# leejaehot/GaussianGrasper

Measured on AMD Instinct MI355X. Metric: rendered views/sec (fwd+bwd) at 1M Gaussians, 1600x1200, 32-ch feature, higher is better.
Workload: dtype f32; 1 GPU; BASELINE config 4 per-GPU share: 1000000 Gaussians, 1600x1200, SH deg 4 rgb + 32-ch feature + depth + normal images per view (nerfstudio plugin route: the timed callable is FusedGaussianSplattingModel.get_outputs(camera) of gaussiangrasper_amd.plugin (the class train.sh loads, on stub.py's stand-ins for nerfstudio's base model and Cameras) — one fused rasterize operator per view), fwd+bwd, 8 views; route=plugin, deterministic_backward=False, python_gc=gc.freeze() after the warm-up (bench.freeze_gc), view_pipeline=backward of view k beside forward of view k + 1 on two streams, num_gaussians=1000000, feature_dim=32, n_visible=992125, parallelism=view-parallel x1, replicated Gaussians, grad_allreduce_bytes=472000000, grad_allreduce=per parameter, overlapped with the last view's backward

## Files before the change

### gaussiangrasper_amd/_lib.py

```python
from __future__ import annotations

import ctypes as C
import os

_HERE = os.path.dirname(os.path.abspath(__file__))
LIB_PATH = os.path.join(_HERE, "libgg_raster.so")
ABI_VERSION = 6

_P, _I, _F, _I64, _SZ = C.c_void_p, C.c_int, C.c_float, C.c_int64, C.c_size_t


class RowArray(C.Structure):
    _fields_ = [("src", C.c_void_p), ("dst", C.c_void_p), ("row_floats", C.c_int), ("kind", C.c_int)]


class AdamGroup(C.Structure):
    _fields_ = [("param", C.c_void_p), ("grad", C.c_void_p), ("exp_avg", C.c_void_p),
                ("exp_avg_sq", C.c_void_p), ("numel", C.c_int64), ("lr", C.c_double),
                ("beta1", C.c_double), ("beta2", C.c_double), ("eps", C.c_double),
                ("weight_decay", C.c_double), ("step", C.c_int64)]


ROWS_COPY, ROWS_MEANS, ROWS_SCALES, ROWS_ZERO_NEW = 0, 1, 2, 3
MAX_ROW_ARRAYS, ADAM_MAX_GROUPS = 24, 8
# ... 12 lines not shown
                               _P, _I, _P, _P, _P]),
    "gg_sh_fwd": (_I, [_I, _I, _I, _P, _P, _P, _P]),
    "gg_sh_bwd": (_I, [_I, _I, _I, _P, _P, _P, _P]),
    "gg_sh_bwd_accumulate": (_I, [_I, _I, _I, _P, _P, _P, _P]),
    "gg_quat_to_rotmat_fwd": (_I, [_I, _P, _P, _P]),
    "gg_quat_to_rotmat_bwd": (_I, [_I, _P, _P, _P, _P]),
    "gg_activate_fwd": (_I, [_I] + [_P] * 12),
    "gg_activate_bwd": (_I, [_I] + [_P] * 12),
    "gg_activate_bwd_ex": (_I, [_I] + [_P] * 7 + [_I] + [_P] * 4 + [_I, _P]),
    "gg_mlp_fwd": (_I, [_I64, _I, _I, _I, _P, _P, _P, _P, _P, _P, _P]),
    "gg_debug_set_fwd_blocks": (_I, [_I, _I]),
    "gg_mlp_fwd_fast_workspace": (_SZ, [_I, _I, _I]),
    "gg_mlp_fwd_fast": (_I, [_I64, _I, _I, _I, _P, _P, _P, _P, _P, _P, _P, _SZ, _P]),
    "gg_mlp_bwd": (_I, [_I64, _I, _I, _I] + [_P] * 11),
    "gg_cosine_loss_fwd": (_I, [_I64, _I, _P, _P, _P, _P, _P, _P, _P]),
    "gg_cosine_loss_bwd": (_I, [_I64, _I, _P, _P, _P, _P, _P, _P, _P, _P, _P]),
    "gg_count_workspace": (_SZ, [_I]),
    "gg_count_intersects": (_I, [_I, _P, _P, _P, _SZ, _P]),
    "gg_bin_sort_workspace": (_SZ, [_I, _I64]),
    "gg_bin_sort": (_I, [_I, _I64, _P, _P, _P, _P, _I, _I, _P, _P, _P, _P, _SZ, _P]),
    "gg_bin_sort_status": (_I, [_I, _I64, _P, _SZ, _P]),
    "gg_bin_sort_dev": (_I, [_I, _I64, _P, _P, _P, _P, _P, _I, _I, _P, _P, _P, _P, _SZ, _P]),
    "gg_bin_sort_dev_ex": (_I, [_I, _I64, _P, _P, _P, _P, _P, _I, _I, _P, _P, _P, _P, _SZ, _P, _P, _I, _P]),
    "gg_view_fwd_workspace": (_SZ, [_I]),
    "gg_view_fwd": (_I, [_I, _P, _P, _P, _P, _P, _P, _P, _F, _F, _F, _F, _I, _I, _I, _I, _F] + [_P] * 11 +
                    [_P, _P, _SZ, _P, _SZ, _P]),
    "gg_blend_fwd_pair_packed": (_I, [_I, _I, _I, _I, _I] + [_P] * 11 + [_SZ, _I, _P]),
    "gg_blend_workspace": (_SZ, [_I]),
    "gg_blend_fwd": (_I, [_I, _I, _I, _I, _P, _P, _P, _P, _P, _P, _P, _P, _P, _P, _P, _SZ, _P]),
    "gg_blend_fwd_pair": (_I, [_I, _I, _I, _I, _I] + [_P] * 14 + [_SZ, _P]),
    "gg_blend_fwd_pair_fast": (_I, [_I, _I, _I, _I, _I] + [_P] * 14 + [_SZ, _P]),
    "gg_blend_bwd": (_I, [_I, _I, _I, _I] + [_P] * 14 + [_I, _I, _P, _SZ, _I, _P]),
    "gg_shade_tail_bwd_split": (_I, [_I, _P, _I, _P, _P, _P, _P, _P]),
    "gg_view_bwd": (_I, [_I, _P, _I, _P, _P, _P, _F, _P, _P, _P, _P, _P, _P, _F, _F, _I, _I, _P, _P, _P, _P, _P, _P, _P, _P]),
    "gg_pose_grad_workspace": (_SZ, [_I]),
    "gg_view_bwd_pose": (_I, [_I, _P, _I, _P, _P, _P, _F, _P, _P, _P, _P, _P, _P, _F, _F, _I, _I] + [_P] * 9
                         + [_P, _SZ, _P]),
    "gg_project_pose_bwd": (_I, [_I, _P, _P, _F, _P, _P, _P, _F, _F, _I, _I, _P, _P, _P, _I, _P, _P, _I, _P, _P, _P,
                                 _SZ, _P]),
    "gg_sh_bwd_multi": (_I, [_I, _I, _I, _I, C.POINTER(_P), C.POINTER(_P), _P, _I, _P]),
    "gg_image_loss_workspace": (_SZ, [_I, _I]),
    "gg_image_loss_fwd": (_I, [_I, _I, _P, _I, _P, _P, _F, _P, _P, _SZ, _P]),
    "gg_image_loss_bwd": (_I, [_I, _I, _P, _I, _P, _P, _F, _P, _P, _SZ, _P, _P]),
    "gg_geom_loss_workspace": (_SZ, []),
    "gg_geom_loss_fwd": (_I, [_I64, _P, _I, _P, _I, _P, _I, _I, _P, _I, _I, _P, _P, _P, _SZ, _P]),
    "gg_geom_loss_bwd": (_I, [_I64, _P, _I, _P, _I, _P, _I, _I, _P, _I, _I, _P, _P, _P, _P, _SZ, _P, _P, _P]),
# ... 101 lines not shown
```

### gaussiangrasper_amd/csrc/binning.hip

```cpp
#include "scan.h"

__device__ __forceinline__ int64_t dev_count(int64_t n, const int64_t *__restrict__ n_dev) {
    if (n_dev) {
        const int64_t d = *n_dev;
        if (d < n) n = d;
    }
    return n;
}

#define RS_THREADS 256
#define RS_WAVES (RS_THREADS / GG_WAVE)
#ifndef GG_RS_BIG
#define GG_RS_BIG 16
#endif
static inline int rs_items(int64_t n) { return n >= (int64_t)4096 * 1024 ? GG_RS_BIG : 4; }

__global__ __launch_bounds__(256) void count_kernel(int N, const int32_t *__restrict__ nth,
                                                    unsigned long long *__restrict__ out) {
    __shared__ unsigned long long part[4];
    unsigned long long acc = 0;
    for (int i = blockIdx.x * blockDim.x + threadIdx.x; i < N; i += gridDim.x * blockDim.x)
        acc += (unsigned long long)(uint32_t)nth[i];
    for (int off = 32; off > 0; off >>= 1) acc += __shfl_down(acc, off, 64);
    if ((threadIdx.x & 63) == 0) part[threadIdx.x >> 6] = acc;
// ... 239 lines not shown
    for (int i = blockIdx.x * 256 + threadIdx.x; i < N; i += 4 * stride) {
        uint32_t k[4];
#pragma unroll
        for (int u = 0; u < 4; ++u) k[u] = (i + u * stride < N) ? depth_key(dsrc, i + u * stride) : 0xFFFFFFFFu;
#pragma unroll
        for (int u = 0; u < 4; ++u)
            if (k[u] != 0xFFFFFFFFu) { lo = min(lo, k[u]); hi = max(hi, k[u]); }
    }
    for (int off = 32; off > 0; off >>= 1) {
        lo = min(lo, (uint32_t)__shfl_xor((int)lo, off, 64));
        hi = max(hi, (uint32_t)__shfl_xor((int)hi, off, 64));
    }
    if ((threadIdx.x & 63) == 0) { s_lo[threadIdx.x >> 6] = lo; s_hi[threadIdx.x >> 6] = hi; }
    __syncthreads();
    if (threadIdx.x == 0) {
        mm[blockIdx.x] = min(min(s_lo[0], s_lo[1]), min(s_lo[2], s_lo[3]));
        mm[gridDim.x + blockIdx.x] = max(max(s_hi[0], s_hi[1]), max(s_hi[2], s_hi[3]));
    }
}
#define DB_BOX_MAX 1023
struct DbGeom {
    const float *xys;
    int tiles_x, tiles_y;
};
__device__ __forceinline__ void db_box(const DbGeom g, const DepthSrc d, int i, uint32_t &cnt, uint32_t &box) {
    const int rad = d.radii[i];
    cnt = 0u;
    box = 1u << 20;
    if (rad > 0) {
        int x0, y0, x1, y1;
        gg_tile_bbox(g.xys[2 * (size_t)i], g.xys[2 * (size_t)i + 1], (float)rad, g.tiles_x, g.tiles_y, x0, y0, x1, y1);
        const int bw = x1 - x0;
        if (bw > 0 && y1 > y0) {
            cnt = (uint32_t)(bw * (y1 - y0));
            box = (uint32_t)x0 | ((uint32_t)y0 << 10) | ((uint32_t)bw << 20);
        }
    }
}
template <bool SCATTER>
__global__ __launch_bounds__(DB_THREADS) void db_walk_kernel(int N, int nb, DepthSrc dsrc, DbGeom geom,
                                                             const DbParts mm, uint32_t *__restrict__ G,
                                                             const uint32_t *__restrict__ start, uint4 *__restrict__ recs,
                                                             int32_t *__restrict__ zero = nullptr, int nzero = 0) {
    for (int i = blockIdx.x * DB_THREADS + threadIdx.x; i < nzero; i += DB_BLOCKS * DB_THREADS) zero[i] = 0;
    extern __shared__ uint32_t s_hist[];
    uint32_t *s_mm = s_hist + nb + 1;
    const DbRange r = db_range_of(mm, nb, s_mm);
    const int per = (N + DB_BLOCKS - 1) / DB_BLOCKS;
    const int lo = blockIdx.x * per, hi = min(N, lo + per);
    uint32_t *row = G + (size_t)blockIdx.x * (nb + 1);
    for (int b = threadIdx.x; b <= nb; b += DB_THREADS) s_hist[b] = SCATTER ? start[b] + row[b] : 0u;
    __syncthreads();
    for (int i = lo + threadIdx.x; i < hi; i += 4 * DB_THREADS) {
        uint32_t k[4], cnt[4], box[4];
// ... 12 lines not shown
                    recs[pos] = make_uint4(k[u], (uint32_t)(i + u * DB_THREADS), cnt[u], box[u]);
            }
        }
    }
    if (!SCATTER) {
        __syncthreads();
        for (int b = threadIdx.x; b <= nb; b += DB_THREADS) row[b] = s_hist[b];
    }
}
__global__ __launch_bounds__(256) void db_prefix_kernel(int nb, uint32_t *__restrict__ G, uint32_t *__restrict__ total) {
    const int b = blockIdx.x * 256 + threadIdx.x;
    if (b > nb) return;
    uint32_t run = 0;
    uint32_t c[DB_BLOCKS];
#pragma unroll
    for (int k = 0; k < DB_BLOCKS; ++k) c[k] = G[(size_t)k * (nb + 1) + b];
#pragma unroll
    for (int k = 0; k < DB_BLOCKS; ++k) {
        G[(size_t)k * (nb + 1) + b] = run;
        run += c[k];
    }
    total[b] = run;
}
__global__ __launch_bounds__(1024) void db_scan_kernel(int n, uint32_t *__restrict__ v) {
    __shared__ uint32_t s_w[2][16];
    const int tid = threadIdx.x, lane = tid & 63, wave = tid >> 6;
    uint32_t carry = 0u;
    int round = 0;
    for (int base = 0; base < n; base += 4 * 4096) {
        uint32_t x[4][4];
#pragma unroll
        for (int q = 0; q < 4; ++q)
#pragma unroll
            for (int k = 0; k < 4; ++k) {
                const int i = base + 4096 * q + 4 * tid + k;
                x[q][k] = i < n ? v[i] : 0u;
            }
#pragma unroll
        for (int q = 0; q < 4; ++q, ++round) {
            if (base + 4096 * q >= n) break;
            const uint32_t mine = x[q][0] + x[q][1] + x[q][2] + x[q][3];
            uint32_t incl = mine;
#pragma unroll
            for (int off = 1; off < 64; off <<= 1) {
                const uint32_t t = __shfl_up(incl, off, 64);
                if (lane >= off) incl += t;
            }
            uint32_t *sw = s_w[round & 1];
            if (lane == 63) sw[wave] = incl;
            __syncthreads();
            uint32_t ex = carry + incl - mine, all = 0u;
#pragma unroll
            for (int w = 0; w < 16; ++w) {
                const uint32_t t = sw[w];
                if (w < wave) ex += t;
                all += t;
            }
            carry += all;
#pragma unroll
            for (int k = 0; k < 4; ++k) {
                const int i = base + 4096 * q + 4 * tid + k;
                if (i < n) v[i] = ex;
                ex += x[q][k];
            }
        }
    }
    if (tid == 0) v[n] = carry;
}

__device__ __forceinline__ void db_ce(u64 &a, u64 &b) {
    const bool sw = b < a;
    const u64 lo = sw ? b : a, hi = sw ? a : b;
    a = lo;
    b = hi;
}
__device__ __forceinline__ void db_bitonic64(u64 *buf, const int n) {
    constexpr int NB = 8, LNB = 3, THREADS = 64;
    const int tid = threadIdx.x & 63;
    int P = NB;
    while (P < n) P <<= 1;
    const u64 INF = ~0ull;
    for (int blk = tid; blk * NB < n; blk += THREADS) {
        u64 v[NB];
#pragma unroll
        for (int r = 0; r < NB; ++r) v[r] = (NB * blk + r < n) ? buf[NB * blk + r] : INF;
#pragma unroll
        for (int k = 2; k <= NB; k <<= 1) {
#pragma unroll
            for (int i = 0; i < NB / 2; ++i) {
                const int b2 = i / (k / 2), off = i % (k / 2);
// ... 406 lines not shown
static void radix_pass(int64_t n, const int64_t *n_dev, const uint32_t *kin, const uint32_t *vin,
                       uint32_t *kout, uint32_t *vout, int shift, uint32_t mask, BinWs &w, hipStream_t s,
                       DepthSrc dsrc = DepthSrc{nullptr, nullptr}) {
    int nb = radix_nblocks(n);
    if (rs_items(n) != 4)
        hipLaunchKernelGGL(radix_hist_kernel<GG_RS_BIG>, dim3(nb), dim3(RS_THREADS), 0, s, n, n_dev, kin, shift,
                           mask, nb, w.G, dsrc);
    else
        hipLaunchKernelGGL(radix_hist_kernel<4>, dim3(nb), dim3(RS_THREADS), 0, s, n, n_dev, kin, shift,
                           mask, nb, w.G, dsrc);
    hipLaunchKernelGGL(radix_colscan_kernel, dim3(256), dim3(256), 0, s, nb, w.G, w.totals);
    if (rs_items(n) != 4)
        hipLaunchKernelGGL(radix_scatter_kernel<GG_RS_BIG>, dim3(nb), dim3(RS_THREADS), 0, s, n, n_dev, kin, vin,
                           kout, vout, shift, mask, nb, w.G, w.totals, dsrc);
    else
        hipLaunchKernelGGL(radix_scatter_kernel<4>, dim3(nb), dim3(RS_THREADS), 0, s, n, n_dev, kin, vin,
                           kout, vout, shift, mask, nb, w.G, w.totals, dsrc);
}

static int bin_sort_impl(int N, int64_t I, const int64_t *I_dev, const float *xys, const float *depths,
                         const int32_t *radii, const int32_t *num_tiles_hit, int tiles_x, int tiles_y,
                         int32_t *gaussian_ids_sorted, int32_t *tile_bins, int32_t *isect_tile_sorted,
                         void *ws, size_t ws_bytes, gg_stream_t stream, const uint32_t *range_lo = nullptr,
                         const uint32_t *range_hi = nullptr, int range_parts = 0) {
    GG_REQUIRE(N >= 0 && I >= 0, "negative size");
    GG_REQUIRE(tiles_x > 0 && tiles_y > 0, "empty tile grid");
    GG_REQUIRE(tiles_x <= DB_BOX_MAX && tiles_y <= DB_BOX_MAX, "tile grid beyond 1023 x 1023 (images beyond 16 368 pixels a side)");
    GG_REQUIRE(I < (int64_t)1 << 31, "num_intersects must fit int32 (tile_bins are int32)");
    GG_REQUIRE(tile_bins != nullptr, "null tile_bins");
    hipStream_t s = (hipStream_t)stream;
    const int T = tiles_x * tiles_y;
    if (N == 0 || I == 0) {
        if (gg_fill_async(tile_bins, 0, sizeof(int32_t) * 2 * (size_t)T, s) != hipSuccess) {
            gg_set_error("gg_bin_sort: memset failed");
            return GG_ERR_LAUNCH;
        }
        return GG_OK;
    }
    GG_REQUIRE(xys && depths && radii && num_tiles_hit && gaussian_ids_sorted, "null pointer");
    BinWs w = bin_ws_layout(ws, N, I);
    if (ws == nullptr || ws_bytes < w.bytes) {
        gg_set_error("gg_bin_sort: workspace too small (%zu < %zu)", ws_bytes, w.bytes);
        return GG_ERR_WORKSPACE;
    }
    gg_prof_begin(GG_K_BIN_SORT, s);
    const int nbk = db_buckets(N);
    const DepthSrc dsrc{depths, radii};
    const size_t walk_lds = sizeof(uint32_t) * ((size_t)nbk + 1 + 2);
    if (walk_lds > 64 * 1024) {
        (void)hipFuncSetAttribute((const void *)db_walk_kernel<false>, hipFuncAttributeMaxDynamicSharedMemorySize, (int)walk_lds);
        (void)hipFuncSetAttribute((const void *)db_walk_kernel<true>, hipFuncAttributeMaxDynamicSharedMemorySize, (int)walk_lds);
    }
    uint32_t *order = w.order;
    DbParts mm{w.dbmm, w.dbmm + 256, 256};
    if (range_lo && range_hi && range_parts > 0)
        mm = DbParts{range_lo, range_hi, range_parts};
    else
        hipLaunchKernelGGL(db_range_kernel, dim3(256), dim3(256), 0, s, N, dsrc, w.dbmm);
    const DbGeom geom{xys, tiles_x, tiles_y};
    hipLaunchKernelGGL(db_walk_kernel<false>, dim3(DB_BLOCKS), dim3(DB_THREADS), walk_lds, s, N, nbk, dsrc, geom, mm,
                       w.dbG, (const uint32_t *)nullptr, (uint4 *)nullptr, tile_bins, 2 * T);
    hipLaunchKernelGGL(db_prefix_kernel, dim3((nbk + 1 + 255) / 256), dim3(256), 0, s, nbk, w.dbG, w.dbStart);
    hipLaunchKernelGGL(db_scan_kernel, dim3(1), dim3(1024), 0, s, nbk, w.dbStart);
    hipLaunchKernelGGL(db_walk_kernel<true>, dim3(DB_BLOCKS), dim3(DB_THREADS), walk_lds, s, N, nbk, dsrc, geom, mm,
                       w.dbG, (const uint32_t *)w.dbStart, w.recs, (int32_t *)nullptr, 0);
    hipLaunchKernelGGL(db_sort_kernel, dim3((nbk + DB_WPB - 1) / DB_WPB), dim3(64 * DB_WPB), 0, s, N, nbk,
                       (const uint32_t *)w.dbStart, (const uint4 *)w.recs, w.pairs, dsrc, geom, order, w.einfo, w.dbBase);
    hipLaunchKernelGGL(db_scan_kernel, dim3(1), dim3(1024), 0, s, nbk, w.dbBase);
    int tile_bits = 1;
    while ((1 << tile_bits) < T) ++tile_bits;
    int passes = (tile_bits + 7) / 8;
    uint32_t *out_vals = (uint32_t *)gaussian_ids_sorted;
    uint32_t *kcur = w.tkeyA, *kalt = w.tkeyB;
    uint32_t *vcur = (passes % 2 == 0) ? out_vals : w.tvalTmp;
    uint32_t *valt = (passes % 2 == 0) ? w.tvalTmp : out_vals;
    if (!I_dev) {
        (void)gg_fill_async(kcur, 0xFF, sizeof(uint32_t) * (size_t)I, s);
        (void)gg_fill_async(vcur, 0, sizeof(uint32_t) * (size_t)I, s);
    }
    hipLaunchKernelGGL(emit_kernel, dim3((N + 255) / 256), dim3(256), 0, s, N, (const uint32_t *)order,
                       (const uint4 *)w.einfo, (const uint32_t *)w.dbBase, (const uint32_t *)(w.dbStart + nbk), tiles_x, I,
                       I_dev, kcur, vcur);
    const int per_pass = (tile_bits + passes - 1) / passes;
    for (int pass = 0; pass < passes; ++pass) {
        int bits = min(per_pass, tile_bits - per_pass * pass);
        radix_pass(I, I_dev, kcur, vcur, kalt, valt, per_pass * pass, (1u << bits) - 1u, w, s);
        uint32_t *t = kcur; kcur = kalt; kalt = t;
        t = vcur; vcur = valt; valt = t;
    }
    hipLaunchKernelGGL(tile_bins_kernel, dim3((unsigned)((I + 255) / 256)), dim3(256), 0, s, I, I_dev, kcur,
                       (uint32_t)T, tile_bins, isect_tile_sorted);
// ... 27 lines not shown
                               const int32_t *num_tiles_hit, int tiles_x, int tiles_y,
                               int32_t *gaussian_ids_sorted, int32_t *tile_bins,
                               int32_t *isect_tile_sorted, void *ws, size_t ws_bytes,
                               gg_stream_t stream) {
    GG_REQUIRE(num_intersects_dev != nullptr, "null num_intersects_dev");
    GG_REQUIRE(capacity >= 1, "capacity < 1");
    return bin_sort_impl(N, capacity, num_intersects_dev, xys, depths, radii, num_tiles_hit, tiles_x,
                         tiles_y, gaussian_ids_sorted, tile_bins, isect_tile_sorted, ws, ws_bytes, stream);
}

extern "C" int gg_bin_sort_dev_ex(int N, int64_t capacity, const int64_t *num_intersects_dev,
                                  const float *xys, const float *depths, const int32_t *radii,
                                  const int32_t *num_tiles_hit, int tiles_x, int tiles_y,
                                  int32_t *gaussian_ids_sorted, int32_t *tile_bins,
                                  int32_t *isect_tile_sorted, void *ws, size_t ws_bytes,
                                  const uint32_t *depth_bits_min, const uint32_t *depth_bits_max, int range_parts,
                                  gg_stream_t stream) {
    GG_REQUIRE(num_intersects_dev != nullptr, "null num_intersects_dev");
    GG_REQUIRE(capacity >= 1, "capacity < 1");
    GG_REQUIRE(range_parts == 0 || (depth_bits_min && depth_bits_max && range_parts > 0), "range parts without arrays");
    return bin_sort_impl(N, capacity, num_intersects_dev, xys, depths, radii, num_tiles_hit, tiles_x,
                         tiles_y, gaussian_ids_sorted, tile_bins, isect_tile_sorted, ws, ws_bytes, stream,
                         depth_bits_min, depth_bits_max, range_parts);
}

size_t gg_sort_pairs_workspace(int64_t n) {
    const size_t i = (size_t)(n > 0 ? n : 1);
    return gg_align_up(4 * i, 256) * 2 + gg_align_up(4 * 256 * (size_t)(radix_nblocks(n) + 1), 256) +
           gg_align_up(4 * 256, 256);
}
int gg_sort_pairs(int64_t n, uint32_t *keys, uint32_t *vals, int bits, void *ws, size_t ws_bytes, hipStream_t s) {
    if (n <= 0) return GG_OK;
    if (ws == nullptr || ws_bytes < gg_sort_pairs_workspace(n)) return GG_ERR_WORKSPACE;
    char *p = (char *)ws;
    const size_t i = (size_t)n;
    uint32_t *kalt = (uint32_t *)p;
    p += gg_align_up(4 * i, 256);
    uint32_t *valt = (uint32_t *)p;
    p += gg_align_up(4 * i, 256);
    BinWs w;
    w.G = (uint32_t *)p;
    p += gg_align_up(4 * 256 * (size_t)(radix_nblocks(n) + 1), 256);
    w.totals = (uint32_t *)p;
    uint32_t *kc = keys, *vc = vals, *ka = kalt, *va = valt;
    const int passes = (bits + 7) / 8;
    for (int pass = 0; pass < passes; ++pass) {
// ... 12 lines not shown
```

### gaussiangrasper_amd/ops.py

```python
from __future__ import annotations

import ctypes as C
from typing import NamedTuple, Optional, Tuple

import torch
from torch import Tensor
from torch.autograd import Function

from . import _lib
from ._call import (f32 as _f32, i32 as _i32, ptr as _ptr, require_hip as _require_hip,
                    stream as _stream, workspace as _workspace)
from .constants import BLOCK, CLIP_THRESH_DEFAULT, deg_from_sh, num_sh_bases


class KeptView(NamedTuple):
    degrees_to_use: int
    num_bases: int
    viewdirs: Tensor
    v_rgb: Tensor


_grad_sinks = {}
_kept_sh = {}

# ... 50 lines not shown
                                               views, v_rgbs, _ptr(buf), 1, _stream(buf.device)), "gg_sh_bwd_multi")
        sink.done()


def _dense_f32(t: Tensor) -> bool:
    return t.dtype == torch.float32 and t.is_contiguous()


def _sink_for(t: Tensor, eligible: bool = True) -> Optional[GradSink]:
    hit = _grad_sinks.get(id(t)) if eligible else None
    return hit if hit is not None and hit.param is t else None


def _sinks_for_all(*tensors: Tensor):
    sinks = [_sink_for(t, _dense_f32(t)) for t in tensors]
    return sinks if all(k is not None for k in sinks) else None


_PIN_SLOTS = 64
_pin_ring = {}
_pending_counts = {}


def _start_count(num_tiles_hit: Tensor, total: Optional[Tensor] = None, depth_parts=None) -> None:
    dev = num_tiles_hit.device
    lib = _lib.load()
    ring, nxt = _pin_ring.get(dev.index, (None, 0))
    if ring is None:
        ring = torch.empty(_PIN_SLOTS, dtype=torch.int64).pin_memory()
    slot = ring[nxt:nxt + 1]
    _pin_ring[dev.index] = (ring, (nxt + 1) % _PIN_SLOTS)
    if total is None:
        total = torch.empty(1, dtype=torch.int64, device=dev)
        _lib.check(lib.gg_count_intersects(num_tiles_hit.shape[0], _ptr(num_tiles_hit), _ptr(total), None, 0,
                                           _stream(dev)), "gg_count_intersects")
    slot.copy_(total, non_blocking=True)
    ev = torch.cuda.Event()
    ev.record(torch.cuda.current_stream(dev))
    if len(_pending_counts) > 8:
        _pending_counts.clear()
    _pending_counts[(num_tiles_hit.data_ptr(), num_tiles_hit._version)] = (ev, slot, num_tiles_hit, total, depth_parts)


def _pending(num_tiles_hit: Tensor):
    hit = _pending_counts.get((num_tiles_hit.data_ptr(), num_tiles_hit._version))
    if hit is None or hit[2] is not num_tiles_hit:
        return None
    return hit


def _take_count(num_tiles_hit: Tensor):
    hit = _pending(num_tiles_hit)
    if hit is None:
        return None
    _pending_counts.pop((num_tiles_hit.data_ptr(), num_tiles_hit._version), None)
    ev, slot = hit[0], hit[1]
    ev.synchronize()
    return int(slot.item())


class ProjectGaussians(Function):
# ... 261 lines not shown
        def redo(b: Binning) -> bool:
            count = _take_count(num_tiles_hit)
            if count is None:
                count = int(total_dev.item())
            _note_count(dev, count)
            b.num_intersects = count
            if count <= cap:
                b.gaussian_ids_sorted = ids[:count]
                return False
            bin_cache_stats["rebinned"] += 1
            b.gaussian_ids_sorted = exact(count)
            return True

        out = Binning(None, ids, tile_bins, key, keep, redo)
    else:
        num_intersects = _take_count(num_tiles_hit)
        if num_intersects is None:
            total = torch.empty(1, dtype=torch.int64, device=dev)
            _lib.check(lib.gg_count_intersects(n, _ptr(nth_c), _ptr(total), None, 0, _stream(dev)),
                       "gg_count_intersects")
            num_intersects = int(total.item())
        _note_count(dev, num_intersects)
        out = Binning(num_intersects, exact(num_intersects), tile_bins, key, keep)
    if use_cache:
        _bin_cache = out
    return out


def _blend_with_lists(bins: Binning, launch) -> bool:
    for attempt in range(2):
        if bins.num_intersects is not None and bins.num_intersects < 1:
            return False
        launch()
        if not bins.resolve():
            break
    return bins.num_intersects >= 1


def _rasterize_forward(ctx, xys, depths, radii, conics, num_tiles_hit, colors, opacity,
                       img_height, img_width, background, three_channel_only):
    if colors.dtype == torch.uint8:
        colors = colors.float() / 255
    if background is not None:
        assert background.shape[0] == colors.shape[-1], \
            f"incorrect shape of background color tensor, expected shape {colors.shape[-1]}"
    else:
# ... 350 lines not shown


class RasterizeSegments(Function):

    @staticmethod
    def forward(ctx, xys, depths, radii, conics, num_tiles_hit, opacity, img_height, img_width, splits, *segs):
        if len(segs) < 2 or len(segs) % 2:
            raise ValueError("expected colors_0, background_0[, colors_1, background_1, ...]")
        if xys.ndimension() != 2 or xys.size(1) != 2:
            raise ValueError("xys must have dimensions (N, 2)")
        if opacity.ndimension() != 2 or opacity.size(1) != 1:
            raise ValueError("opacity must have dimensions (N, 1)")
        cols, bgs = list(segs[0::2]), list(segs[1::2])
        dev = _require_hip(xys, depths, radii, conics, num_tiles_hit, opacity, *cols, *bgs)
        n = xys.size(0)
        img_height, img_width = int(img_height), int(img_width)
        for c, b in zip(cols, bgs):
            if c.ndimension() != 2 or c.size(0) != n:
                raise ValueError("colors must have dimensions (N, D)")
            assert b.shape[0] == c.shape[1], f"incorrect shape of background color tensor, expected shape {c.shape[1]}"
        xys_c, conics_c, opacity_c = _f32(xys), _f32(conics), _f32(opacity)
        cols_c, bgs_c = [_f32(c) for c in cols], [_f32(b) for b in bgs]
        ctx.sinks = [_sink_for(c, c.shape[1] > 8 and _dense_f32(c)) for c in cols]
        bins = bin_and_sort_gaussians(xys, depths, radii, num_tiles_hit, img_height, img_width, speculative=True)
        lib = _lib.load()
        packed = None
        if isinstance(splits, tuple) and len(splits) == 2 and (splits[1] is None or isinstance(splits[1], Tensor)) \
                and isinstance(splits[0], tuple):
            splits, packed = splits
        if packed is not None and (packed.dtype != torch.uint8 or packed.numel() < lib.gg_blend_workspace(n)
                                   or packed.device != dev):
            raise ValueError("packed: a uint8 blend workspace of gg_blend_workspace(N) bytes on the operands' device")
        ws = packed if packed is not None else _workspace(lib.gg_blend_workspace(n), dev)
        final_Ts = torch.empty(img_height, img_width, dtype=torch.float32, device=dev)
        final_idx = torch.empty(img_height, img_width, dtype=torch.int32, device=dev)
        outs = [torch.empty(img_height, img_width, c.shape[1], dtype=torch.float32, device=dev) for c in cols_c]
        wide = next((i for i, c in enumerate(cols_c) if c.shape[1] >= 32), None)
        small = next((i for i, c in enumerate(cols_c) if c.shape[1] <= 8), None) if wide is not None else None

        def launch():
            if small is not None and packed is not None:
                _lib.check(lib.gg_blend_fwd_pair_packed(
                    cols_c[wide].shape[1], cols_c[small].shape[1], n, img_height, img_width,
                    _ptr(bins.gaussian_ids_sorted), _ptr(bins.tile_bins), _ptr(cols_c[wide]), _ptr(cols_c[small]),
                    _ptr(bgs_c[wide]), _ptr(bgs_c[small]), _ptr(outs[wide]), _ptr(outs[small]), _ptr(final_Ts),
                    _ptr(final_idx), _ptr(ws), ws.numel(), 0 if (EXACT_FORWARD or _DETERMINISTIC) else 1,
                    _stream(dev)), "gg_blend_fwd_pair_packed")
            elif small is not None:
                pair_fwd = lib.gg_blend_fwd_pair if (EXACT_FORWARD or _DETERMINISTIC) else lib.gg_blend_fwd_pair_fast
                _lib.check(pair_fwd(
                    cols_c[wide].shape[1], cols_c[small].shape[1], n, img_height, img_width,
                    _ptr(bins.gaussian_ids_sorted), _ptr(bins.tile_bins), _ptr(xys_c), _ptr(conics_c),
# ... 107 lines not shown
            sink = ctx.sinks[i]
            if i == rider:
                v_colors, cstride = rec_g[:, 6:gwidth], gstride
            elif sink is not None:
                v_colors, cstride = sink.buffer, 0
                flags |= 2
            else:
                v_colors, cstride = torch.empty(n, ch, dtype=torch.float32, device=dev), 0
            _blend_bwd(lib, ch, n, img_height, img_width, ids_sorted, tile_bins, xys, conics, cols[i], opacity,
                       bgs[i], final_Ts, final_idx, v_out, v_xy, v_conic, v_colors, v_opacity, gstride, cstride,
                       ws, flags, ctx.num_intersects)
            first = False
            if flags & 2:
                sink.done()
            else:
                grads[i] = v_colors
        seg_grads = []
        for g in grads:
            seg_grads += [g, None]
        return (v_xy, None, None, v_conic, None, v_opacity.reshape(ctx.opacity_shape), None, None, None, *seg_grads)


def rasterize_segments(xys, depths, radii, conics, num_tiles_hit, opacity, img_height, img_width, segments,
                       packed: Optional[Tensor] = None):
    flat, splits = [], {}
    for i, seg in enumerate(segments):
        flat += [seg[0], seg[1]]
        if len(seg) > 2 and seg[2] is not None:
            splits[i] = tuple(int(x) for x in seg[2])
    spec = tuple(sorted(splits.items()))
    return list(RasterizeSegments.apply(xys, depths, radii, conics, num_tiles_hit, opacity, img_height,
                                        img_width, (spec, packed) if packed is not None else spec, *flat))


class _QuatToRotmat(Function):
    @staticmethod
    def forward(ctx, quat: Tensor) -> Tensor:
        dev = _require_hip(quat)
        q = _f32(quat).reshape(-1, 4)
        rot = torch.empty(q.shape[0], 9, dtype=torch.float32, device=dev)
        _lib.check(_lib.load().gg_quat_to_rotmat_fwd(q.shape[0], _ptr(q), _ptr(rot), _stream(dev)),
                   "gg_quat_to_rotmat_fwd")
        ctx.save_for_backward(q)
        ctx.in_shape, ctx.in_dtype = quat.shape, quat.dtype
        return rot.reshape(quat.shape[:-1] + (3, 3))

    @staticmethod
    def backward(ctx, v_rot: Tensor):
        (q,) = ctx.saved_tensors
        dev = q.device
        g = _f32(v_rot).reshape(-1, 9)
        v_q = torch.empty_like(q)
        _lib.check(_lib.load().gg_quat_to_rotmat_bwd(q.shape[0], _ptr(q), _ptr(g), _ptr(v_q),
                                                     _stream(dev)), "gg_quat_to_rotmat_bwd")
        return v_q.reshape(ctx.in_shape).to(ctx.in_dtype)
# ... 7 lines not shown
```

### gaussiangrasper_amd/pipeline.py

```python
from __future__ import annotations

from typing import Callable, Dict, Union

import torch

from .camera import ViewParams
from .scene import Scene

CHANNELS = ("rgb", "feature", "depth", "normal")


def smallest_axis_normals(quats: torch.Tensor, log_scales: torch.Tensor, quat_to_rotmat) -> torch.Tensor:
    rot = quat_to_rotmat(quats)
    idx = log_scales.exp().min(dim=-1)[1][..., None, None].expand(-1, 3, -1)
    return rot.gather(2, idx).squeeze(dim=2)


def activate(scene: Scene, view: ViewParams, quat_to_rotmat) -> Dict[str, Union[torch.Tensor, Callable]]:
    viewdirs = scene.means.detach() - view.cam_pos.to(scene.means.device)
    viewdirs = viewdirs / viewdirs.norm(dim=-1, keepdim=True)
    return {
        "means": scene.means,
        "scales": torch.exp(scene.scales),
        "quats": scene.quats / scene.quats.norm(dim=-1, keepdim=True),
# ... 46 lines not shown
    return out


_CONSTANTS: Dict = {}


def _zeros(d: int, dev) -> torch.Tensor:
    key = ("zeros", d, str(dev))
    if key not in _CONSTANTS:
        _CONSTANTS[key] = torch.zeros(d, device=dev)
    return _CONSTANTS[key]


def _tail_background(dev) -> torch.Tensor:
    key = ("tail", str(dev))
    if key not in _CONSTANTS:
        bg = torch.zeros(7, device=dev)
        bg[3] = 10.0
        _CONSTANTS[key] = bg
    return _CONSTANTS[key]


def fused_images(ops, xys, depths, radii, conics, num_tiles_hit, opac, h, w, feature, rgbs, normals, tail=None,
                 packed=None):
    dev = xys.device
    d = feature.shape[1]
    if hasattr(ops, "rasterize_segments"):
        if tail is None:
            tail = torch.cat([rgbs, depths[:, None], normals], dim=1)
        bg_tail = _tail_background(dev)
        kw = {"packed": packed} if packed is not None else {}
        feat_im, rgb, depth, normal = ops.rasterize_segments(
            xys, depths, radii, conics, num_tiles_hit, opac, h, w,
            [(feature, _zeros(d, dev)), (tail, bg_tail, (3, 1, 3))], **kw)
        return feat_im, rgb, depth, normal
    colors = torch.cat([feature, rgbs, depths[:, None], normals], dim=1)
    background = torch.zeros(d + 7, device=dev)
    background[d + 3] = 10.0
    img = ops.NDRasterizeGaussians.apply(xys, depths, radii, conics, num_tiles_hit, colors, opac, h, w,
                                         background)
    return torch.split(img, [d, 3, 1, 3], dim=-1)


def rasterize_activated_fused(act: Dict, view: ViewParams, ops, sh_degree_to_use: int = 4
                              ) -> Dict[str, torch.Tensor]:
    dev = act["means"].device
    h, w = view.height, view.width
    opac = act["opac"]() if callable(act["opac"]) else act["opac"]
    xys, depths, radii, conics, num_tiles_hit, cov3d = ops.ProjectGaussians.apply(
        act["means"], act["scales"], 1, act["quats"], view.viewmat[:3, :].to(dev),
        view.projmat.to(dev), view.fx, view.fy, view.cx, view.cy, h, w, view.tile_bounds)
    if xys.requires_grad:
        xys.retain_grad()
    if hasattr(ops, "ShadeTail") and hasattr(ops, "rasterize_segments"):
# ... 35 lines not shown
```

### gaussiangrasper_amd/plugin.py

```python
from __future__ import annotations

import copy
import math
from typing import Dict, List, Optional, Union

import torch

from . import ops as _ops
from .camera import projection_matrix
from .constants import BLOCK
from .pipeline import fused_images

DESCRIPTION = ("GaussianGrasper feature-field splatting on the MI355X-native fused rasterizer "
               "(gaussiangrasper_amd): one rasterize call per view for rgb + feature + depth + normal")


def fused_view(model, means, log_scales, quats, opacities, colors_all, feature, viewmat, projmat, cam_pos,
               fx, fy, cx, cy, H, W, tile_bounds, sh_degree_to_use: int, ops=_ops, full_proj=None
               ) -> Optional[Dict[str, torch.Tensor]]:
    if hasattr(ops, "ViewGeometry") and hasattr(ops, "rasterize_segments") and model.config.sh_degree > 0:
        if full_proj is None:
            full_proj = projmat @ viewmat
        model._gg_last_view = (viewmat, full_proj)
        model.xys, depths, model.radii, conics, num_tiles_hit, opac, tail, model.normals, packed = ops.ViewGeometry.apply(
            means, log_scales, quats, opacities, colors_all, cam_pos.reshape(-1)[:3], viewmat[:3, :], full_proj,
            fx, fy, cx, cy, H, W, tile_bounds, sh_degree_to_use)
        if model.training:
            model.xys.retain_grad()
        feat_im, rgb, depth_im, normal_im = fused_images(ops, model.xys, depths, model.radii, conics, num_tiles_hit,
                                                         opac, H, W, feature, None, model.normals, tail=tail,
                                                         packed=packed)
        count = ops.last_num_intersects(model.radii)
        if count == 0 or (count is None and (model.radii).sum() == 0):
            return None
        return {"rgb": rgb, "feature": feat_im, "depth": depth_im, "normal": normal_im}
    fused_act = hasattr(ops, "ActivateGaussians")
    if fused_act:
        scales_e, quats_n, opac, viewdirs, model.normals = ops.ActivateGaussians.apply(
            means, log_scales, quats, opacities, cam_pos.reshape(-1)[:3])
    else:
        scales_e, quats_n = torch.exp(log_scales), quats / quats.norm(dim=-1, keepdim=True)
        opac = torch.sigmoid(opacities)
    if full_proj is None:
        full_proj = projmat @ viewmat
    model._gg_last_view = (viewmat, full_proj)
    model.xys, depths, model.radii, conics, num_tiles_hit, _cov3d = ops.ProjectGaussians.apply(
        means, scales_e, 1, quats_n, viewmat[:3, :], full_proj, fx, fy, cx, cy, H, W, tile_bounds)
    count_known_late = hasattr(ops, "last_num_intersects")
    if not count_known_late and (model.radii).sum() == 0:
        return None
    if model.training:
        model.xys.retain_grad()
    if not fused_act:
        rot = ops.quat_to_rotmat(quats)
# ... 441 lines not shown
```

### include/gg_raster.h

```cpp
#ifndef GG_RASTER_H
#define GG_RASTER_H

#include <stddef.h>
#include <stdint.h>

#ifdef __cplusplus
extern "C" {
#endif

#define GG_OK 0
#define GG_ERR_INVALID_ARG (-1)
#define GG_ERR_LAUNCH (-2)
#define GG_ERR_WORKSPACE (-3)
#define GG_ERR_UNSUPPORTED (-4)

typedef void *gg_stream_t;

int gg_abi_version(void);
const char *gg_last_error(void);

int gg_project_fwd(int num_points, const float *means3d, const float *scales, float glob_scale,
                   const float *quats, const float *viewmat, const float *projmat, float fx,
                   float fy, float cx, float cy, int img_height, int img_width, int tiles_x,
                   int tiles_y, float clip_thresh, float *cov3d, float *xys, float *depths,
// ... 84 lines not shown

size_t gg_count_workspace(int num_points);
int gg_count_intersects(int num_points, const int32_t *num_tiles_hit,
                        int64_t *num_intersects_out, void *ws, size_t ws_bytes,
                        gg_stream_t stream);

size_t gg_bin_sort_workspace(int num_points, int64_t num_intersects);
int gg_bin_sort(int num_points, int64_t num_intersects, const float *xys, const float *depths,
                const int32_t *radii, const int32_t *num_tiles_hit, int tiles_x, int tiles_y,
                int32_t *gaussian_ids_sorted, int32_t *tile_bins, int32_t *isect_tile_sorted,
                void *ws, size_t ws_bytes, gg_stream_t stream);

int gg_bin_sort_status(int num_points, int64_t num_intersects, const void *ws, size_t ws_bytes, gg_stream_t stream);
int gg_bin_sort_dev(int num_points, int64_t capacity, const int64_t *num_intersects_dev,
                    const float *xys, const float *depths, const int32_t *radii,
                    const int32_t *num_tiles_hit, int tiles_x, int tiles_y,
                    int32_t *gaussian_ids_sorted, int32_t *tile_bins, int32_t *isect_tile_sorted,
                    void *ws, size_t ws_bytes, gg_stream_t stream);
int gg_bin_sort_dev_ex(int num_points, int64_t capacity, const int64_t *num_intersects_dev, const float *xys,
                       const float *depths, const int32_t *radii, const int32_t *num_tiles_hit, int tiles_x, int tiles_y,
                       int32_t *gaussian_ids_sorted, int32_t *tile_bins, int32_t *isect_tile_sorted, void *ws,
                       size_t ws_bytes, const uint32_t *depth_bits_min, const uint32_t *depth_bits_max, int range_parts,
                       gg_stream_t stream);

size_t gg_blend_workspace(int num_points);
int gg_blend_fwd(int channels, int num_points, int img_height, int img_width,
                 const int32_t *gaussian_ids_sorted, const int32_t *tile_bins, const float *xys,
                 const float *conics, const float *colors, const float *opacity,
                 const float *background, float *out_img, float *final_Ts, int32_t *final_idx,
                 void *ws, size_t ws_bytes, gg_stream_t stream);

int gg_blend_fwd_pair(int channels, int channels2, int num_points, int img_height, int img_width,
                      const int32_t *gaussian_ids_sorted, const int32_t *tile_bins, const float *xys,
                      const float *conics, const float *colors, const float *colors2,
                      const float *opacity, const float *background, const float *background2,
                      float *out_img, float *out_img2, float *final_Ts, int32_t *final_idx, void *ws,
                      size_t ws_bytes, gg_stream_t stream);

int gg_blend_fwd_pair_fast(int channels, int channels2, int num_points, int img_height, int img_width,
                           const int32_t *gaussian_ids_sorted, const int32_t *tile_bins, const float *xys,
                           const float *conics, const float *colors, const float *colors2,
                           const float *opacity, const float *background, const float *background2,
                           float *out_img, float *out_img2, float *final_Ts, int32_t *final_idx, void *ws,
                           size_t ws_bytes, gg_stream_t stream);
int gg_blend_fwd_pair_packed(int channels, int channels2, int num_points, int img_height, int img_width,
                             const int32_t *gaussian_ids_sorted, const int32_t *tile_bins, const float *colors,
// ... 294 lines not shown
```

Measured before the change: 632.4 views/s.

## Bin Gaussians into tiles using tight ellipse extents from packed blend records

Adds a tight binning path that intersects each Gaussian's radius-based tile box with a box derived from its conic and alpha threshold, taken from the packed blend records. Gaussians that can never pass the threshold are dropped. This cuts the number of tile intersections that are sorted and blended in both forward and backward. The true intersection count is now produced on the device by the scan kernel and read back through the pinned ring, with a speculative capacity and a re-bin when it is exceeded. The path is on by default in the plugin, and the risk is that extents too tight against the blend kernel's cutoff would drop contributions.

```diff
diff --git a/gaussiangrasper_amd/_lib.py b/gaussiangrasper_amd/_lib.py
--- a/gaussiangrasper_amd/_lib.py
+++ b/gaussiangrasper_amd/_lib.py
@@ -58,6 +58,7 @@
     "gg_bin_sort_status": (_I, [_I, _I64, _P, _SZ, _P]),
     "gg_bin_sort_dev": (_I, [_I, _I64, _P, _P, _P, _P, _P, _I, _I, _P, _P, _P, _P, _SZ, _P]),
     "gg_bin_sort_dev_ex": (_I, [_I, _I64, _P, _P, _P, _P, _P, _I, _I, _P, _P, _P, _P, _SZ, _P, _P, _I, _P]),
+    "gg_bin_sort_tight": (_I, [_I, _I64, _P, _P, _P, _P, _I, _I, _P, _P, _P, _P, _P, _SZ, _P, _P, _I, _P]),
     "gg_view_fwd_workspace": (_SZ, [_I]),
     "gg_view_fwd": (_I, [_I, _P, _P, _P, _P, _P, _P, _P, _F, _F, _F, _F, _I, _I, _I, _I, _F] + [_P] * 11 +
                     [_P, _P, _SZ, _P, _SZ, _P]),
diff --git a/gaussiangrasper_amd/csrc/binning.hip b/gaussiangrasper_amd/csrc/binning.hip
--- a/gaussiangrasper_amd/csrc/binning.hip
+++ b/gaussiangrasper_amd/csrc/binning.hip
@@ -1,4 +1,5 @@
 #include "scan.h"
+#include "blend_common.h"
 
 __device__ __forceinline__ int64_t dev_count(int64_t n, const int64_t *__restrict__ n_dev) {
     if (n_dev) {
@@ -285,7 +286,22 @@
 struct DbGeom {
     const float *xys;
     int tiles_x, tiles_y;
+    const GRec *rec;
 };
+__device__ __forceinline__ bool db_tight_range(const GRec r, int tiles_x, int tiles_y, int &x0, int &y0, int &x1, int &y1) {
+    const float ac = r.ca * r.cc, bb = r.cb * r.cb;
+    const float det = (ac - bb) - 2.4e-7f * (ac + bb);
+    if (!(r.ca > 0.0f) || !(r.cc > 0.0f) || !(det > 0.0f) || !(r.thr < __builtin_inff()) || !(r.thr >= 0.0f)) return false;
+    const float hx0 = sqrtf(2.0f * r.thr * r.cc / det), hy0 = sqrtf(2.0f * r.thr * r.ca / det);
+    const float hx = hx0 + (1e-5f * (hx0 + fabsf(r.x)) + 1e-4f), hy = hy0 + (1e-5f * (hy0 + fabsf(r.y)) + 1e-4f);
+    const float px0 = ceilf(r.x - hx), px1 = floorf(r.x + hx), py0 = ceilf(r.y - hy), py1 = floorf(r.y + hy);
+    if (!(px0 == px0) || !(px1 == px1) || !(py0 == py0) || !(py1 == py1)) return false;
+    x0 = gg_clampi_f(px0 * (1.0f / GG_BLOCK), tiles_x);
+    x1 = (px1 < 0.0f || px1 < px0) ? 0 : gg_clampi_f(px1 * (1.0f / GG_BLOCK) + 1.0f, tiles_x);
+    y0 = gg_clampi_f(py0 * (1.0f / GG_BLOCK), tiles_y);
+    y1 = (py1 < 0.0f || py1 < py0) ? 0 : gg_clampi_f(py1 * (1.0f / GG_BLOCK) + 1.0f, tiles_y);
+    return true;
+}
 __device__ __forceinline__ void db_box(const DbGeom g, const DepthSrc d, int i, uint32_t &cnt, uint32_t &box) {
     const int rad = d.radii[i];
     cnt = 0u;
@@ -293,6 +309,15 @@
     if (rad > 0) {
         int x0, y0, x1, y1;
         gg_tile_bbox(g.xys[2 * (size_t)i], g.xys[2 * (size_t)i + 1], (float)rad, g.tiles_x, g.tiles_y, x0, y0, x1, y1);
+        if (g.rec) {
+            const GRec r = g.rec[i];
+            if (r.thr < 0.0f) return;
+            int tx0, ty0, tx1, ty1;
+            if (db_tight_range(r, g.tiles_x, g.tiles_y, tx0, ty0, tx1, ty1)) {
+                x0 = max(x0, tx0); y0 = max(y0, ty0);
+                x1 = min(x1, tx1); y1 = min(y1, ty1);
+            }
+        }
         const int bw = x1 - x0;
         if (bw > 0 && y1 > y0) {
             cnt = (uint32_t)(bw * (y1 - y0));
@@ -351,7 +376,7 @@
     }
     total[b] = run;
 }
-__global__ __launch_bounds__(1024) void db_scan_kernel(int n, uint32_t *__restrict__ v) {
+__global__ __launch_bounds__(1024) void db_scan_kernel(int n, uint32_t *__restrict__ v, int64_t *__restrict__ total64 = nullptr) {
     __shared__ uint32_t s_w[2][16];
     const int tid = threadIdx.x, lane = tid & 63, wave = tid >> 6;
     uint32_t carry = 0u;
@@ -394,7 +419,10 @@
             }
         }
     }
-    if (tid == 0) v[n] = carry;
+    if (tid == 0) {
+        v[n] = carry;
+        if (total64) *total64 = (int64_t)carry;
+    }
 }
 
 __device__ __forceinline__ void db_ce(u64 &a, u64 &b) {
@@ -847,7 +875,8 @@
                          const int32_t *radii, const int32_t *num_tiles_hit, int tiles_x, int tiles_y,
                          int32_t *gaussian_ids_sorted, int32_t *tile_bins, int32_t *isect_tile_sorted,
                          void *ws, size_t ws_bytes, gg_stream_t stream, const uint32_t *range_lo = nullptr,
-                         const uint32_t *range_hi = nullptr, int range_parts = 0) {
+                         const uint32_t *range_hi = nullptr, int range_parts = 0, const GRec *tight_rec = nullptr,
+                         int64_t *tight_count = nullptr) {
     GG_REQUIRE(N >= 0 && I >= 0, "negative size");
     GG_REQUIRE(tiles_x > 0 && tiles_y > 0, "empty tile grid");
     GG_REQUIRE(tiles_x <= DB_BOX_MAX && tiles_y <= DB_BOX_MAX, "tile grid beyond 1023 x 1023 (images beyond 16 368 pixels a side)");
@@ -856,13 +885,14 @@
     hipStream_t s = (hipStream_t)stream;
     const int T = tiles_x * tiles_y;
     if (N == 0 || I == 0) {
-        if (gg_fill_async(tile_bins, 0, sizeof(int32_t) * 2 * (size_t)T, s) != hipSuccess) {
+        if (gg_fill_async(tile_bins, 0, sizeof(int32_t) * 2 * (size_t)T, s) != hipSuccess ||
+            (tight_count && gg_fill_async(tight_count, 0, sizeof(int64_t), s) != hipSuccess)) {
             gg_set_error("gg_bin_sort: memset failed");
             return GG_ERR_LAUNCH;
         }
         return GG_OK;
     }
-    GG_REQUIRE(xys && depths && radii && num_tiles_hit && gaussian_ids_sorted, "null pointer");
+    GG_REQUIRE(xys && depths && radii && (num_tiles_hit || tight_rec) && gaussian_ids_sorted, "null pointer");
     BinWs w = bin_ws_layout(ws, N, I);
     if (ws == nullptr || ws_bytes < w.bytes) {
         gg_set_error("gg_bin_sort: workspace too small (%zu < %zu)", ws_bytes, w.bytes);
@@ -882,16 +912,16 @@
         mm = DbParts{range_lo, range_hi, range_parts};
     else
         hipLaunchKernelGGL(db_range_kernel, dim3(256), dim3(256), 0, s, N, dsrc, w.dbmm);
-    const DbGeom geom{xys, tiles_x, tiles_y};
+    const DbGeom geom{xys, tiles_x, tiles_y, tight_rec};
     hipLaunchKernelGGL(db_walk_kernel<false>, dim3(DB_BLOCKS), dim3(DB_THREADS), walk_lds, s, N, nbk, dsrc, geom, mm,
                        w.dbG, (const uint32_t *)nullptr, (uint4 *)nullptr, tile_bins, 2 * T);
     hipLaunchKernelGGL(db_prefix_kernel, dim3((nbk + 1 + 255) / 256), dim3(256), 0, s, nbk, w.dbG, w.dbStart);
-    hipLaunchKernelGGL(db_scan_kernel, dim3(1), dim3(1024), 0, s, nbk, w.dbStart);
+    hipLaunchKernelGGL(db_scan_kernel, dim3(1), dim3(1024), 0, s, nbk, w.dbStart, (int64_t *)nullptr);
     hipLaunchKernelGGL(db_walk_kernel<true>, dim3(DB_BLOCKS), dim3(DB_THREADS), walk_lds, s, N, nbk, dsrc, geom, mm,
                        w.dbG, (const uint32_t *)w.dbStart, w.recs, (int32_t *)nullptr, 0);
     hipLaunchKernelGGL(db_sort_kernel, dim3((nbk + DB_WPB - 1) / DB_WPB), dim3(64 * DB_WPB), 0, s, N, nbk,
                        (const uint32_t *)w.dbStart, (const uint4 *)w.recs, w.pairs, dsrc, geom, order, w.einfo, w.dbBase);
-    hipLaunchKernelGGL(db_scan_kernel, dim3(1), dim3(1024), 0, s, nbk, w.dbBase);
+    hipLaunchKernelGGL(db_scan_kernel, dim3(1), dim3(1024), 0, s, nbk, w.dbBase, tight_count);
     int tile_bits = 1;
     while ((1 << tile_bits) < T) ++tile_bits;
     int passes = (tile_bits + 7) / 8;
@@ -965,6 +995,20 @@
     return bin_sort_impl(N, capacity, num_intersects_dev, xys, depths, radii, num_tiles_hit, tiles_x,
                          tiles_y, gaussian_ids_sorted, tile_bins, isect_tile_sorted, ws, ws_bytes, stream,
                          depth_bits_min, depth_bits_max, range_parts);
+}
+
+extern "C" int gg_bin_sort_tight(int N, int64_t capacity, const float *xys, const float *depths, const int32_t *radii,
+                                 const void *records, int tiles_x, int tiles_y, int32_t *gaussian_ids_sorted,
+                                 int32_t *tile_bins, int32_t *isect_tile_sorted, int64_t *num_intersects_out, void *ws,
+                                 size_t ws_bytes, const uint32_t *depth_bits_min, const uint32_t *depth_bits_max,
+                                 int range_parts, gg_stream_t stream) {
+    GG_REQUIRE(num_intersects_out != nullptr, "null num_intersects_out");
+    GG_REQUIRE(capacity >= 1, "capacity < 1");
+    GG_REQUIRE(N <= 0 || (records != nullptr && ((uintptr_t)records & 15) == 0), "records: null or not 16-byte aligned");
+    GG_REQUIRE(range_parts == 0 || (depth_bits_min && depth_bits_max && range_parts > 0), "range parts without arrays");
+    return bin_sort_impl(N, capacity, num_intersects_out, xys, depths, radii, nullptr, tiles_x, tiles_y,
+                         gaussian_ids_sorted, tile_bins, isect_tile_sorted, ws, ws_bytes, stream, depth_bits_min,
+                         depth_bits_max, range_parts, (const GRec *)records, num_intersects_out);
 }
 
 size_t gg_sort_pairs_workspace(int64_t n) {
diff --git a/gaussiangrasper_amd/ops.py b/gaussiangrasper_amd/ops.py
--- a/gaussiangrasper_amd/ops.py
+++ b/gaussiangrasper_amd/ops.py
@@ -96,21 +96,27 @@
 _pending_counts = {}
 
 
-def _start_count(num_tiles_hit: Tensor, total: Optional[Tensor] = None, depth_parts=None) -> None:
-    dev = num_tiles_hit.device
-    lib = _lib.load()
+def _read_back(total: Tensor):
+    dev = total.device
     ring, nxt = _pin_ring.get(dev.index, (None, 0))
     if ring is None:
         ring = torch.empty(_PIN_SLOTS, dtype=torch.int64).pin_memory()
     slot = ring[nxt:nxt + 1]
     _pin_ring[dev.index] = (ring, (nxt + 1) % _PIN_SLOTS)
+    slot.copy_(total, non_blocking=True)
+    ev = torch.cuda.Event()
+    ev.record(torch.cuda.current_stream(dev))
+    return ev, slot
+
+
+def _start_count(num_tiles_hit: Tensor, total: Optional[Tensor] = None, depth_parts=None) -> None:
+    dev = num_tiles_hit.device
+    lib = _lib.load()
     if total is None:
         total = torch.empty(1, dtype=torch.int64, device=dev)
         _lib.check(lib.gg_count_intersects(num_tiles_hit.shape[0], _ptr(num_tiles_hit), _ptr(total), None, 0,
                                            _stream(dev)), "gg_count_intersects")
-    slot.copy_(total, non_blocking=True)
-    ev = torch.cuda.Event()
-    ev.record(torch.cuda.current_stream(dev))
+    ev, slot = _read_back(total)
     if len(_pending_counts) > 8:
         _pending_counts.clear()
     _pending_counts[(num_tiles_hit.data_ptr(), num_tiles_hit._version)] = (ev, slot, num_tiles_hit, total, depth_parts)
@@ -418,6 +424,74 @@
             num_intersects = int(total.item())
         _note_count(dev, num_intersects)
         out = Binning(num_intersects, exact(num_intersects), tile_bins, key, keep)
+    if use_cache:
+        _bin_cache = out
+    return out
+
+
+def bin_tight(xys: Tensor, depths: Tensor, radii: Tensor, num_tiles_hit: Tensor, records: Tensor,
+              img_height: int, img_width: int, use_cache: bool = True) -> Binning:
+    global _bin_cache
+    dev = _require_hip(xys, depths, radii, num_tiles_hit, records)
+    key = _bin_key(xys, depths, radii, num_tiles_hit, img_height, img_width) + ("tight", records.data_ptr())
+    if use_cache and _bin_cache is not None and _bin_cache.key == key:
+        bin_cache_stats["hits"] += 1
+        return _bin_cache
+    bin_cache_stats["misses"] += 1
+    lib = _lib.load()
+    n = xys.shape[0]
+    if records.dtype != torch.uint8 or records.numel() < lib.gg_blend_workspace(n):
+        raise ValueError("records: a uint8 blend workspace of gg_blend_workspace(N) bytes")
+    tiles_x = (img_width + BLOCK - 1) // BLOCK
+    tiles_y = (img_height + BLOCK - 1) // BLOCK
+    xys_c, depths_c, radii_c = _f32(xys.detach()), _f32(depths.detach()), _i32(radii)
+    tile_bins = torch.empty(tiles_x * tiles_y, 2, dtype=torch.int32, device=dev)
+    keep = (xys, depths, radii, num_tiles_hit, records)
+    pending = _pending(num_tiles_hit)
+    parts = pending[4] if pending is not None else None
+
+    def run(cap: int):
+        ids = torch.empty(cap, dtype=torch.int32, device=dev)
+        total_dev = torch.empty(1, dtype=torch.int64, device=dev)
+        ws = _workspace(lib.gg_bin_sort_workspace(n, cap), dev)
+        _lib.check(lib.gg_bin_sort_tight(n, cap, _ptr(xys_c), _ptr(depths_c), _ptr(radii_c), _ptr(records), tiles_x,
+                                         tiles_y, _ptr(ids), _ptr(tile_bins), None, _ptr(total_dev), _ptr(ws),
+                                         ws.numel(), _ptr(parts[0]) if parts else None,
+                                         _ptr(parts[1]) if parts else None, parts[2] if parts else 0, _stream(dev)),
+                   "gg_bin_sort_tight")
+        return ids, total_dev
+
+    cap = _capacity_hint.get(dev.index, 0)
+    if pending is not None and cap > 0:
+        bin_cache_stats["speculative"] += 1
+        ids, total_dev = run(cap)
+        ev, slot = _read_back(total_dev)
+        _pending_counts.pop((num_tiles_hit.data_ptr(), num_tiles_hit._version), None)
+
+        def redo(b: Binning) -> bool:
+            ev.synchronize()
+            count = int(slot.item())
+            _note_count(dev, count)
+            b.num_intersects = count
+            if count <= cap:
+                b.gaussian_ids_sorted = ids[:count]
+                return False
+            bin_cache_stats["rebinned"] += 1
+            b.gaussian_ids_sorted = run(count)[0][:count]
+            return True
+
+        out = Binning(None, ids, tile_bins, key, keep, redo)
+    else:
+        upper = _take_count(num_tiles_hit)
+        if upper is None:
+            total = torch.empty(1, dtype=torch.int64, device=dev)
+            _lib.check(lib.gg_count_intersects(n, _ptr(_i32(num_tiles_hit)), _ptr(total), None, 0, _stream(dev)),
+                       "gg_count_intersects")
+            upper = int(total.item())
+        ids, total_dev = run(max(upper, 1))
+        count = int(total_dev.item())
+        _note_count(dev, count)
+        out = Binning(count, ids[:count], tile_bins, key, keep)
     if use_cache:
         _bin_cache = out
     return out
@@ -814,12 +888,17 @@
         xys_c, conics_c, opacity_c = _f32(xys), _f32(conics), _f32(opacity)
         cols_c, bgs_c = [_f32(c) for c in cols], [_f32(b) for b in bgs]
         ctx.sinks = [_sink_for(c, c.shape[1] > 8 and _dense_f32(c)) for c in cols]
-        bins = bin_and_sort_gaussians(xys, depths, radii, num_tiles_hit, img_height, img_width, speculative=True)
         lib = _lib.load()
-        packed = None
-        if isinstance(splits, tuple) and len(splits) == 2 and (splits[1] is None or isinstance(splits[1], Tensor)) \
+        packed, tight = None, False
+        if isinstance(splits, tuple) and len(splits) in (2, 3) and (splits[1] is None or isinstance(splits[1], Tensor)) \
                 and isinstance(splits[0], tuple):
-            splits, packed = splits
+            splits, packed, tight = splits[0], splits[1], len(splits) == 3 and bool(splits[2])
+        if tight and packed is None:
+            raise ValueError("tight_lists needs the packed records the lists are cut from (packed=...)")
+        if tight:
+            bins = bin_tight(xys, depths, radii, num_tiles_hit, packed, img_height, img_width)
+        else:
+            bins = bin_and_sort_gaussians(xys, depths, radii, num_tiles_hit, img_height, img_width, speculative=True)
         if packed is not None and (packed.dtype != torch.uint8 or packed.numel() < lib.gg_blend_workspace(n)
                                    or packed.device != dev):
             raise ValueError("packed: a uint8 blend workspace of gg_blend_workspace(N) bytes on the operands' device")
@@ -973,7 +1052,7 @@
 
 
 def rasterize_segments(xys, depths, radii, conics, num_tiles_hit, opacity, img_height, img_width, segments,
-                       packed: Optional[Tensor] = None):
+                       packed: Optional[Tensor] = None, tight_lists: bool = False):
     flat, splits = [], {}
     for i, seg in enumerate(segments):
         flat += [seg[0], seg[1]]
@@ -981,7 +1060,8 @@
             splits[i] = tuple(int(x) for x in seg[2])
     spec = tuple(sorted(splits.items()))
     return list(RasterizeSegments.apply(xys, depths, radii, conics, num_tiles_hit, opacity, img_height,
-                                        img_width, (spec, packed) if packed is not None else spec, *flat))
+                                        img_width, (spec, packed, bool(tight_lists)) if packed is not None else spec,
+                                        *flat))
 
 
 class _QuatToRotmat(Function):
diff --git a/gaussiangrasper_amd/pipeline.py b/gaussiangrasper_amd/pipeline.py
--- a/gaussiangrasper_amd/pipeline.py
+++ b/gaussiangrasper_amd/pipeline.py
@@ -92,7 +92,7 @@
 
 
 def fused_images(ops, xys, depths, radii, conics, num_tiles_hit, opac, h, w, feature, rgbs, normals, tail=None,
-                 packed=None):
+                 packed=None, tight_lists=False):
     dev = xys.device
     d = feature.shape[1]
     if hasattr(ops, "rasterize_segments"):
@@ -100,6 +100,8 @@
             tail = torch.cat([rgbs, depths[:, None], normals], dim=1)
         bg_tail = _tail_background(dev)
         kw = {"packed": packed} if packed is not None else {}
+        if tight_lists and packed is not None:
+            kw["tight_lists"] = True
         feat_im, rgb, depth, normal = ops.rasterize_segments(
             xys, depths, radii, conics, num_tiles_hit, opac, h, w,
             [(feature, _zeros(d, dev)), (tail, bg_tail, (3, 1, 3))], **kw)
diff --git a/gaussiangrasper_amd/plugin.py b/gaussiangrasper_amd/plugin.py
--- a/gaussiangrasper_amd/plugin.py
+++ b/gaussiangrasper_amd/plugin.py
@@ -13,6 +13,15 @@
 
 DESCRIPTION = ("GaussianGrasper feature-field splatting on the MI355X-native fused rasterizer "
                "(gaussiangrasper_amd): one rasterize call per view for rgb + feature + depth + normal")
+
+
+TIGHT_LISTS = True
+
+
+def set_tight_lists(on: bool = True) -> bool:
+    global TIGHT_LISTS
+    prev, TIGHT_LISTS = TIGHT_LISTS, bool(on)
+    return prev
 
 
 def fused_view(model, means, log_scales, quats, opacities, colors_all, feature, viewmat, projmat, cam_pos,
@@ -29,7 +38,7 @@
             model.xys.retain_grad()
         feat_im, rgb, depth_im, normal_im = fused_images(ops, model.xys, depths, model.radii, conics, num_tiles_hit,
                                                          opac, H, W, feature, None, model.normals, tail=tail,
-                                                         packed=packed)
+                                                         packed=packed, tight_lists=TIGHT_LISTS)
         count = ops.last_num_intersects(model.radii)
         if count == 0 or (count is None and (model.radii).sum() == 0):
             return None
diff --git a/include/gg_raster.h b/include/gg_raster.h
--- a/include/gg_raster.h
+++ b/include/gg_raster.h
@@ -130,6 +130,11 @@
                        int32_t *gaussian_ids_sorted, int32_t *tile_bins, int32_t *isect_tile_sorted, void *ws,
                        size_t ws_bytes, const uint32_t *depth_bits_min, const uint32_t *depth_bits_max, int range_parts,
                        gg_stream_t stream);
+int gg_bin_sort_tight(int num_points, int64_t capacity, const float *xys, const float *depths, const int32_t *radii,
+                      const void *records, int tiles_x, int tiles_y, int32_t *gaussian_ids_sorted, int32_t *tile_bins,
+                      int32_t *isect_tile_sorted, int64_t *num_intersects_out, void *ws, size_t ws_bytes,
+                      const uint32_t *depth_bits_min, const uint32_t *depth_bits_max, int range_parts,
+                      gg_stream_t stream);
 
 size_t gg_blend_workspace(int num_points);
 int gg_blend_fwd(int channels, int num_points, int img_height, int img_width,
```

Measured after the change: 633.5 views/s (median of 4 runs). About the same (+0.2%).
